# Maofei/loam_velodyne-1

Measured on AMD Instinct MI355X. Metric: scans/sec (odometry+mapping L-M solve) VLP-16 sweep, 1/2/4/8 MI355X, higher is better.
Workload: dtype fp32 (fp64 JtJ accumulation); 1 GPU; config4: independent VLP-16 problems (SR prev+cur, odometry L-M, mapping L-M); problems_per_gpu=1024, global_batch=1024, split=strong, parallelism=shard1

## Files before the change

loam_velodyne-1_amd/csrc/dev_common.hpp:

```cpp
#ifndef LOAM_DEV_COMMON_HPP
#define LOAM_DEV_COMMON_HPP

#include <hip/hip_runtime.h>
#include <stdint.h>

#define LOAM_HD __host__ __device__ __forceinline__
#define LOAM_D __device__ __forceinline__

#ifdef LOAM_BOUNDS_CHECK
#define LOAM_CHECK(cond, a, b)                                                                      \
  do {                                                                                              \
    if (!(cond)) printf("LOAM_CHECK %s:%d %s (%lld, %lld)\n", __FILE__, __LINE__, #cond, (long long)(a), \
                        (long long)(b));                                                            \
  } while (0)
#else
#define LOAM_CHECK(cond, a, b) ((void)0)
#endif

struct PhaseAcc {
  unsigned long long s0, s1, s2;
  unsigned long long sum[2][12];
};
#ifdef LOAM_PHASES
#define LOAM_PH(...) __VA_ARGS__
// ... 251 lines not shown
    mx[d] = b;
  }
  __syncthreads();
}
template <bool HALF = false>
LOAM_D int wave_incl_scan_x(int v) {
  const uint32_t u = (uint32_t)v;
  uint32_t s = u + dpp_u32<kDppShr1>(0u, u);
  s += dpp_u32<kDppShr2>(0u, u);
  s += dpp_u32<kDppShr3>(0u, u);
  s += dpp_u32<kDppShr4, 0xf, 0xe>(0u, s);
  s += dpp_u32<kDppShr8, 0xf, 0xc>(0u, s);
  s += dpp_u32<kDppBcast15, 0xa, 0xf>(0u, s);
  if constexpr (!HALF) s += dpp_u32<kDppBcast31, 0xc, 0xf>(0u, s);
  return (int)s;
}

LOAM_D int wave_incl_max(int v) {
  for (int o = 1; o < 64; o <<= 1) {
    int w = __shfl_up(v, o, 64);
    if (lane_id() >= o) v = max(v, w);
  }
  return v;
}

template <int NT>
LOAM_D int block_incl_max(int v, int* scratch, int& total) {
  const int nw = NT / 64, w = threadIdx.x >> 6, l = lane_id();
  int incl = wave_incl_max(v);
  if (l == 63) scratch[w] = incl;
// ... 1006 lines not shown
```

loam_velodyne-1_amd/csrc/dev_hooks.h:

```cpp
#ifndef LOAM_DEV_HOOKS_H
#define LOAM_DEV_HOOKS_H

#include <stdint.h>

#ifdef __cplusplus
extern "C" {
#endif

typedef struct loam_dev_vg loam_dev_vg;

#define LOAM_DEV_VG_STACK 0
#define LOAM_DEV_VG_CUBES 1
#define LOAM_DEV_VG_SURROUND 2

typedef struct {
  const float* pts;
  int32_t total;
  int32_t nseg;
  const int32_t* begin;
  const int32_t* end;
  const float* leaf;
  const int32_t* nold;
  int32_t route;
  int32_t P;
// ... 43 lines not shown
typedef struct {
  const float* cloud;
  int32_t n_cloud;
  const float* queries;
  int32_t n_queries;
  const int32_t* seeds;
} loam_dev_od_nn_job;

int loam_dev_od_nn_create(int device, loam_dev_od_nn** out);

int loam_dev_od_nn_run(loam_dev_od_nn* h, const loam_dev_od_nn_job* job, uint64_t* lane_key, uint64_t* wave_key,
                       uint64_t* chunk_key, int32_t* left);

int loam_dev_od_nn_destroy(loam_dev_od_nn* h);

#ifdef __cplusplus
}
#endif
#endif
```

loam_velodyne-1_amd/csrc/engine.cpp:

```cpp
#include <hip/hip_runtime.h>

#include <cstdio>
#include <cstddef>
#include <algorithm>
#include <cmath>
#include <cstring>
#include <string>
#include <thread>
#include <vector>

#include "../../include/loam/loam.h"
#include "engine.hpp"
#include "lanes.hpp"
#include "mp.hpp"
#include "od.hpp"
#include "pose_math.hpp"
#include "score.hpp"

#ifdef LOAM_PIPE_TRACE
namespace {
struct PipeTrace {
  struct Mark { int step; const char* stage; hipEvent_t a, b; };
  std::vector<Mark> marks;
  int step = 0;
// ... 71 lines not shown
  return v;
}

}

constexpr size_t kMetaBytes = 8192;

struct loam_ctx {
  loam_config cfg;
  int device = 0;
  hipStream_t st = nullptr;
  int R = 16, cap = 40000;
  int sr_init_count = 0;
  bool sr_inited = false;
  SrBuffers sr1;
  SrBuffers odin;
  OdBuffers od1;
  bool od_inited = false;
  int od_last = 0, od_frame_count = 1;
  float od_sum[6] = {0, 0, 0, 0, 0, 0};
  MpBuffers mp1;
  int map_frame_count = 4;
  bool surround_due = false;
  loamimu::SrQueue* sr_imu = nullptr;
  loamimu::SrQueue* sr_imu_dev = nullptr;
  loamimu::MpQueue mp_imu;
  double imu_last_stamp = -1e300;
  int P = 0;
  SrBuffers srb;
  SrBuffers srb2;
// ... 170 lines not shown
  return LOAM_OK;
}

int sr_errors(int e) {
  if (e & ERR_EMPTY) return fail(LOAM_E_INVAL, "sweep has no finite point");
  if (e & ERR_CAP_RING) return fail(LOAM_E_CAPACITY, "a ring span exceeds the per-ring capacity");
  return LOAM_OK;
}

SrParams sr_params(const loam_ctx* c) {
  SrParams p;
  p.R = c->R;
  p.ring_model = (int)c->cfg.ring_model;
  p.ring_lo = c->cfg.ring_lo_deg;
  p.ring_hi = c->cfg.ring_hi_deg;
  return p;
}

void count_bytes(loam_stats& s) {
  s.bytes_sr = 16 * s.n_raw + 32 * s.n_ring + 16 * (s.n_sharp + s.n_less_sharp + s.n_flat + s.n_less_flat);
  s.bytes_od = 16 * s.od_assoc_points + 16 * s.od_queries + 12 * s.od_queries + 32 * s.od_rows_sum;
  s.bytes_mp = 16 * s.mp_map_points + 96 * s.mp_stack_iters + 64 * s.mp_rows_sum + 32 * s.mp_stack +
               32 * s.mp_map_valid_points;
}

}

namespace loam {
void set_last_error(const std::string& msg) { g_err = msg; }
}
// ... 60 lines not shown
  if (he == hipSuccess) he = hipEventCreateWithFlags(&x->seed_done, hipEventDisableTiming);
  for (auto& e : x->step_done)
    if (he == hipSuccess) he = hipEventCreateWithFlags(&e, hipEventDisableTiming);
  for (auto& e : x->feed_copied)
    if (he == hipSuccess) he = hipEventCreateWithFlags(&e, hipEventDisableTiming);
  x->pin.streams[0] = x->st;
  x->pin.streams[1] = x->st2;
  if (he == hipSuccess) he = hipEventCreateWithFlags(&x->fork, hipEventDisableTiming);
  if (he == hipSuccess) he = hipEventCreateWithFlags(&x->join, hipEventDisableTiming);
  if (he == hipSuccess) he = hipEventCreateWithFlags(&x->fork2, hipEventDisableTiming);
  if (he == hipSuccess) he = hipEventCreateWithFlags(&x->join2, hipEventDisableTiming);
  if (he != hipSuccess) {
    loam_destroy(x);
    return fail(LOAM_E_HIP, std::string("event creation failed: ") + hipGetErrorString(he));
  }
  if (he == hipSuccess) he = sr_alloc(x->sr1, 1, x->cap, x->R);
  if (he == hipSuccess) he = sr_alloc(x->odin, 1, x->cap, x->R);
  if (he == hipSuccess) he = od_alloc(x->od1, 1, x->R, x->cap, (int)c.od_max_iter);
  if (he == hipSuccess) he = mp_alloc(x->mp1, 1, x->R, x->cap, (int)c.map_capacity, (int)c.mp_max_iter);
  x->od1.tune = x->mp1.tune = x->tune;
  if (he == hipSuccess) he = hipMalloc(&x->sr_imu_dev, sizeof(loamimu::SrQueue));
  if (he != hipSuccess) x->sr_imu_dev = nullptr;
  if (he == hipSuccess) he = hipHostMalloc((void**)&x->meta, kMetaBytes, hipHostMallocDefault);
  if (he != hipSuccess) x->meta = nullptr;
  if (he == hipSuccess) he = hipHostMalloc((void**)&x->xb.h, kXferBytes, hipHostMallocCoherent | hipHostMallocMapped);
  if (he != hipSuccess) x->xb.h = nullptr;
  else std::memset(x->xb.h, 0, kXferBytes);
  if (he == hipSuccess) he = hipHostGetDevicePointer((void**)&x->xb.d, x->xb.h, 0);
  x->sr_imu = new loamimu::SrQueue();
  std::memset(x->sr_imu, 0, sizeof(loamimu::SrQueue));
// ... 4 lines not shown
  if (he != hipSuccess) {
    loam_destroy(x);
    return fail(LOAM_E_NOMEM, std::string("device allocation failed: ") + hipGetErrorString(he));
  }
  *out = x;
  return LOAM_OK;
}

void loam_destroy(loam_ctx* x) {
  if (!x) return;
  (void)hipSetDevice(x->device);
  if (x->st) (void)hipStreamSynchronize(x->st);
  if (x->st2) (void)hipStreamSynchronize(x->st2);
  if (x->st3) (void)hipStreamSynchronize(x->st3);
  if (x->st4) (void)hipStreamSynchronize(x->st4);
  sr_free(x->sr1);
  sr_free(x->odin);
  od_free(x->od1);
  mp_free(x->mp1);
  sr_free(x->srb);
  sr_free(x->srb2);
  sr_free(x->srb3);
  od_free(x->odb);
  mp_free(x->mpb);
  mp_free(x->mpb2);
  x->free_feed();
  x->free_pack();
  mp_map_free(x->mio);
  mp_loc_free(x->loc);
  mp_score_free(x->score);
// ... 2113 lines not shown
```

loam_velodyne-1_amd/csrc/engine.hpp:

```cpp
#ifndef LOAM_ENGINE_HPP
#define LOAM_ENGINE_HPP

#include <hip/hip_runtime.h>
#include <stdint.h>

#include <cstring>
#include <string>

#include "../../include/loam/loam.h"
#include "imu.hpp"
#include "prof.hpp"

namespace loam {

enum : int {
  ERR_CAP_RING = 1,
  ERR_CAP_ROWS = 2,
  ERR_EMPTY = 4,
  ERR_CAP_MAP = 8,
  ERR_CAP_STACK = 16,
  ERR_VG_BITS = 32,
};

constexpr int kSrThreads = 512;
// ... 92 lines not shown
  int* err = nullptr;
  int* sel_big = nullptr;
  int* sel_list = nullptr;
  int* st_loff = nullptr;
  uint64_t* big_keys = nullptr;
  int* big_sidx = nullptr;
  int* big_cand = nullptr;
  int big_stride = 0;
  __host__ __device__ int ntiles() const { return (cap + kSrThreads - 1) / kSrThreads; }
};

struct SrParams {
  int R;
  int ring_model;
  float ring_lo, ring_hi;
  loamimu::SrQueue* imu = nullptr;
  double time_scan = 0.0;
  const loamimu::LaneHdr* imu_lane = nullptr;
  loamimu::SrTail* imu_tail = nullptr;
  int* imu_tile_key = nullptr;
};

struct DevAlloc {
  hipError_t err = hipSuccess;
  template <class T>
  void operator()(T** p, size_t bytes) {
    *p = nullptr;
    if (err != hipSuccess) return;
    void* q = nullptr;
    err = hipMalloc(&q, bytes ? bytes : 16);
// ... 61 lines not shown
  }
  void finish() {
    for (int i = 0; i < nout; ++i) memcpy(out[i].dst, out[i].src, out[i].bytes);
    nout = 0;
  }
  void release() {
    if (buf) (void)hipHostFree(buf);
    buf = nullptr;
    cap = off = 0;
    nout = 0;
  }
};

void set_last_error(const std::string& msg);

hipError_t sr_alloc(SrBuffers& b, int S, int cap, int R);
hipError_t sr_scatter_packed(const float4* src, const int* off, const int* n, float4* raw, int cap, int S,
                             hipStream_t st);
void sr_free(SrBuffers& b);
constexpr int kPackClouds = 5;
hipError_t sr_pack_offsets(const SrBuffers& b, int s0, int ns, uint64_t* table, hipStream_t st);
hipError_t sr_pack(const SrBuffers& b, const uint64_t* table, int s0, int ns, int j0, int nj, unsigned clouds,
                   const long long* dbase, float4* dst, hipStream_t st);
void sr_launch(const SrBuffers& b, const SrParams& p, hipStream_t st, Prof* prof = nullptr,
               hipEvent_t sorted = nullptr);

}

#endif
```

loam_velodyne-1_amd/csrc/sr.hip:

```cpp
#include <type_traits>

#include "dev_common.hpp"
#include "engine.hpp"

using namespace loamdev;

namespace loam {

namespace {


LOAM_D int ring_id(const SrParams& p, float angle) {
  if (p.ring_model == LOAM_RING_LINEAR) {
    const float step = (p.ring_hi - p.ring_lo) / (float)(p.R - 1);
    const float angleID = (angle - p.ring_lo) / step;
    return (int)(angleID + 0.5f);
  }
  int rounded = (int)(D(angle) + (D(angle) < 0.0 ? -0.5 : +0.5));
  return rounded > 0 ? rounded : rounded + (p.R - 1);
}

LOAM_D int ring_of(const SrParams& p, float px, float py, float pz) {
  const float af = atanf(py / sqrtf(px * px + pz * pz)) * 57.2957795f;
  const int lo = ring_id(p, af - 1e-3f), hi = ring_id(p, af + 1e-3f);
  if (lo == hi) return lo;
  return ring_id(p, (float)(atan(D(py) / sqrt(D(px * px + pz * pz))) * 180 / M_PI));
}

using loamimu::kNoOri;
using loamimu::ori_first;
using loamimu::ori_key;
using loamimu::ori_second;
LOAM_D bool finite3(const float4& q) {
  return isfinite(q.x) && isfinite(q.y) && isfinite(q.z);
}

template <bool IMU>
__global__ __launch_bounds__(kSrThreads) void k_sr_ring_sort(SrBuffers b, SrParams p) {
  const int s = blockIdx.x, tid = threadIdx.x, lane = lane_id(), w = tid >> 6;
  const int n = b.raw_n[s];
  const float4* raw = b.raw + (size_t)s * b.cap;
  float* tori = b.tmp_ori + (size_t)s * b.cap;
  uint8_t* tsid = b.tmp_sid + (size_t)s * b.cap;
  const int R = p.R, ntiles = (n + kSrThreads - 1) / kSrThreads;
  int* tc = b.tilecnt + (size_t)s * b.ntiles() * R;
  __shared__ int sh_first, sh_last, sh_F, sh_total;
  __shared__ float sh_start, sh_end;
  __shared__ int sh_cnt[64];
  __shared__ int sh_wcnt[kSrThreads / 64][64];
  __shared__ int sh_base[64];
  if (tid == 0) { sh_first = 0x7fffffff; sh_last = -1; sh_F = 0x7fffffff; }
  __syncthreads();
  int f = 0x7fffffff, l = -1;
  for (int i = tid; i < n; i += kSrThreads) {
    if (finite3(raw[i])) { f = min(f, i); l = max(l, i); }
  }
  f = wave_min_i(f);
  l = wave_max_i(l);
  if (lane == 0) { atomicMin(&sh_first, f); atomicMax(&sh_last, l); }
  __syncthreads();
  if (sh_last < 0) {
    if (tid == 0) { b.n_full[s] = 0; b.err[s] |= ERR_EMPTY; }
    return;
  }
  if (tid == 0) {
// ... 6 lines not shown
    sh_end = endOri;
  }
  __syncthreads();
  const float startOri = sh_start, endOri = sh_end;
  int Floc = 0x7fffffff;
  for (int t = 0; t < ntiles; ++t) {
    if (tid < R) sh_cnt[tid] = 0;
    __syncthreads();
    const int i = t * kSrThreads + tid;
    if (i < n) {
      const float4 q = raw[i];
      uint8_t sid = 255;
      float ori = 0.0f;
      if (finite3(q)) {
        const float px = q.y, py = q.z, pz = q.x;
        int scanID = ring_of(p, px, py, pz);
        if (scanID >= 0 && scanID <= R - 1) {
          sid = (uint8_t)scanID;
          ori = -atan2f_fdlibm(px, pz);
          float o1 = ori_first(ori, startOri);
          if (D(o1 - startOri) > M_PI) Floc = min(Floc, i);
          atomicAdd(&sh_cnt[scanID], 1);
        }
      }
      tori[i] = ori;
      tsid[i] = sid;
    }
    __syncthreads();
    if (tid < R) tc[t * R + tid] = sh_cnt[tid];
    __syncthreads();
  }
// ... 58 lines not shown
        const float ori = (i <= F) ? ori_first(tori[i], startOri) : ori_second(tori[i], endOri);
        const float relTime = (ori - startOri) / (endOri - startOri);
        pointTime = (float)(D(relTime) * 0.1);
        g = loamimu::first_later(*imu, front0, p.time_scan + pointTime);
      }
      int tmax;
      const int incl = block_incl_max<kSrThreads>(g, sh_imuscr, tmax);
      front_i = max(sh_carry, incl);
      __syncthreads();
      if (tid == 0) sh_carry = max(sh_carry, tmax);
    }
    loamimu::Cur cur;
    float fs[6];
    if (lane < R) sh_wcnt[w][lane] = 0;
    __builtin_amdgcn_wave_barrier();
    int rank = 0;
    uint64_t mval = __ballot(valid);
    while (mval) {
      const int leader = __ffsll((unsigned long long)mval) - 1;
      const int rl = __builtin_amdgcn_readlane(sid, leader);
      const uint64_t mm = __ballot(valid && sid == rl);
      if (valid && sid == rl) rank = __popcll(mm & lanemask_lt());
      if (lane == leader) sh_wcnt[w][rl] = __popcll(mm);
      mval &= ~mm;
    }
    __syncthreads();
    if (valid) {
      int pos = sh_base[sid] + tc[t * R + sid] + rank;
      for (int v = 0; v < w; ++v) pos += sh_wcnt[v][sid];
      const float4 q = raw[i];
      float ori = tori[i];
      ori = (i <= F) ? ori_first(ori, startOri) : ori_second(ori, endOri);
      float relTime = (ori - startOri) / (endOri - startOri);
      float4 o;
      o.x = q.y;
      o.y = q.z;
      o.z = q.x;
      o.w = (float)(sid + 0.1 * D(relTime));
      if (imu) {
        cur = loamimu::interpolate(*imu, (front0 + front_i) % loamimu::kQue, p.time_scan, pointTime);
// ... 67 lines not shown
    for (int base = 0; base < n; base += 64) {
      const int i = base + lane;
      const uint64_t m = __ballot(i < n && finite3(raw[i]));
      if (m) { f = base + __ffsll((unsigned long long)m) - 1; break; }
    }
    if (lane == 0) sh_first = f;
  } else if (w == 1) {
    int l = -1;
    for (int base = n - 1; base >= 0; base -= 64) {
      const int i = base - lane;
      const uint64_t m = __ballot(i >= 0 && finite3(raw[i]));
      if (m) { l = base - (__ffsll((unsigned long long)m) - 1); break; }
    }
    if (lane == 0) sh_last = l;
  }
  if (tid < R) sh_cnt[tid] = 0;
  if (tid == 0) sh_F = 0x7fffffff;
  __syncthreads();
  if (tid == 0) sh_start = sh_last >= 0 ? -atan2f_fdlibm(raw[sh_first].y, raw[sh_first].x) : 0.0f;
  if (tid == 64 && (t == 0 || imu) && sh_last >= 0) sh_end_raw = -atan2f_fdlibm(raw[sh_last].y, raw[sh_last].x);
  __syncthreads();
  const float startOri = sh_start;
  if (IMU && imu) {
    if (tid == 0) {
      float endOri = 0.0f;
      if (sh_last >= 0) {
        endOri = (float)(D(sh_end_raw) + 2 * M_PI);
        if (D(endOri - startOri) > 3 * M_PI) endOri = (float)(D(endOri) - 2 * M_PI);
        else if (D(endOri - startOri) < M_PI) endOri = (float)(D(endOri) + 2 * M_PI);
      }
// ... 14 lines not shown
    }
    b.sweep_ori[2 * s] = startOri;
    b.sweep_ori[2 * s + 1] = endOri;
  }
  int Floc = 0x7fffffff;
  int k1[kRingE], k2[kRingE];
#pragma unroll
  for (int e = 0; e < kRingE; ++e) {
    const int i = t * kRingTile + e * kSrThreads + tid;
    k1[e] = k2[e] = kNoOri;
    if (i < n) {
      uint8_t sid = 255;
      float ori = 0.0f;
      if (finite3(q[e])) {
        const float px = q[e].y, py = q[e].z, pz = q[e].x;
        const int scanID = ring_of(p, px, py, pz);
        if (scanID >= 0 && scanID <= R - 1) {
          sid = (uint8_t)scanID;
          ori = -atan2f_fdlibm(px, pz);
          const float o1 = ori_first(ori, startOri);
          if (D(o1 - startOri) > M_PI) Floc = min(Floc, i);
          atomicAdd(&sh_cnt[scanID], 1);
          if (IMU && imu) {
            k1[e] = ori_key(o1);
            k2[e] = ori_key(ori_second(ori, sh_end));
          }
        }
      }
      b.tmp_ori[(size_t)s * b.cap + i] = ori;
      b.tmp_sid[(size_t)s * b.cap + i] = sid;
    }
// ... 13 lines not shown
      else m2 = max(m2, k2[e]);
    }
    m1 = wave_max_i(m1); m2 = wave_max_i(m2); m3 = wave_max_i(m3);
    if (lane == 0) { atomicMax(&sh_key[0], m1); atomicMax(&sh_key[1], m2); atomicMax(&sh_key[2], m3); }
    __syncthreads();
    if (tid < 3) p.imu_tile_key[((size_t)s * b.ntiles() + t) * 3 + tid] = sh_key[tid];
  }
}

template <bool IMU>
__global__ __launch_bounds__(kSrThreads) void k_sr_ring_scatter(SrBuffers b, SrParams p) {
  constexpr int kW = kSrThreads / 64, kSlots = kRingE * kW;
  static_assert(kSlots <= 64 && (kSlots & (kSlots - 1)) == 0, "slot scan width");
  const int s = blockIdx.y, t = blockIdx.x, tid = threadIdx.x, lane = lane_id(), w = tid >> 6;
  const int n = b.raw_n[s], R = p.R, nt = (n + kRingTile - 1) / kRingTile;
  if (t >= (nt > 0 ? nt : 1)) return;
  const bool imu = IMU && p.imu_lane[s].has != 0;
  __shared__ int sh_later;
  __shared__ int sh_tot[64], sh_pre[64], sh_base[64], sh_F;
  __shared__ int sh_wcnt[64][kSlots];
  int sid[kRingE], rank[kRingE];
  float4 q[kRingE];
  float ori[kRingE];
#pragma unroll
  for (int e = 0; e < kRingE; ++e) {
    const int i = t * kRingTile + e * kSrThreads + tid;
    sid[e] = 255;
    q[e] = make_float4(0, 0, 0, 0);
    ori[e] = 0.0f;
    if (i < n) {
// ... 11 lines not shown
  for (int k = tid; k < nt * R; k += kSrThreads) {
    const int v = tc[k];
    if (v) {
      atomicAdd(&sh_tot[k % R], v);
      if (k / R < t) atomicAdd(&sh_pre[k % R], v);
      if (IMU && k / R > t) sh_later = 1;
    }
  }
  int F = 0x7fffffff;
  for (int k = tid; k < nt; k += kSrThreads) F = min(F, b.tileF[(size_t)s * b.ntiles() + k]);
  F = wave_min_i(F);
  if (lane == 0 && F != 0x7fffffff) atomicMin(&sh_F, F);
#pragma unroll
  for (int e = 0; e < kRingE; ++e) {
    const bool valid = sid[e] != 255;
    rank[e] = 0;
    uint64_t mval = __ballot(valid);
    while (mval) {
      const int leader = __ffsll((unsigned long long)mval) - 1;
      const int rl = __builtin_amdgcn_readlane(sid[e], leader);
      const uint64_t mm = __ballot(valid && sid[e] == rl);
      if (valid && sid[e] == rl) rank[e] = __popcll(mm & lanemask_lt());
      if (lane == leader) sh_wcnt[rl][e * kW + w] = __popcll(mm);
      mval &= ~mm;
    }
  }
  __syncthreads();
  if (tid == 0) {
    int run = 0;
    for (int r = 0; r < R; ++r) { sh_base[r] = run; run += sh_tot[r]; }
    if (t == 0) {
      b.n_full[s] = run;
      if (n <= 0) b.err[s] |= ERR_EMPTY;
    }
  }
  for (int k = tid; k < R * kSlots; k += kSrThreads) {
    const int r = k / kSlots, j = k % kSlots;
    const int v = sh_wcnt[r][j];
    int incl = v;
#pragma unroll
// ... 103 lines not shown
}

#ifndef LOAM_SR_RING_FUSED
#define LOAM_SR_RING_FUSED 1
#endif
constexpr bool kSrRingFused = LOAM_SR_RING_FUSED;
constexpr int kSrRingFusedMin = 64;
__global__ __launch_bounds__(kSrThreads) void k_sr_ring_fused(SrBuffers b, SrParams p, int rtiles) {
  constexpr int kW = kSrThreads / 64, kSlots = kRingE * kW;
  static_assert(kSlots <= 64 && (kSlots & (kSlots - 1)) == 0, "slot scan width");
  const int tid = threadIdx.x, lane = lane_id(), w = tid >> 6;
  __shared__ int sh_ticket, sh_last, sh_F;
  __shared__ float sh_start, sh_end_raw;
  __shared__ int sh_cnt[64], sh_tot[64], sh_pre[64], sh_base[64];
  __shared__ int sh_wcnt[64][kSlots];
  if (tid == 0) sh_ticket = atomicAdd(&b.ring_sync[0], 1);
  __syncthreads();
  const int s = sh_ticket / rtiles, t = sh_ticket % rtiles;
  const int n = b.raw_n[s], R = p.R, nt = (n + kRingTile - 1) / kRingTile;
  if (t == 0) {
    if (tid < 2 * R) b.ring_se[s * 2 * R + tid] = 0;
    if (tid == 0) b.err[s] = 0;
  }
  if (n <= 0) {
    if (t == 0 && tid == 0) {
      b.n_full[s] = 0;
      b.err[s] |= ERR_EMPTY;
    }
    return;
  }
  if (t >= nt) return;
  const float4* raw = b.raw + (size_t)s * b.cap;
  float4 q[kRingE];
#pragma unroll
// ... 14 lines not shown
        f = w == 0 ? k + src : n - 1 - k - src;
        v.x = __shfl(v.x, src, 64);
        v.y = __shfl(v.y, src, 64);
        break;
      }
    }
    if (lane == 0) {
      if (w == 0) {
        sh_start = f >= 0 ? -atan2f_fdlibm(v.y, v.x) : 0.0f;
      } else {
        sh_last = f;
        if (f >= 0) sh_end_raw = -atan2f_fdlibm(v.y, v.x);
      }
    }
  }
  if (tid < R) sh_cnt[tid] = 0;
  if (tid == 0) sh_F = 0x7fffffff;
  for (int k = tid; k < 64 * kSlots; k += kSrThreads) (&sh_wcnt[0][0])[k] = 0;
  __syncthreads();
  const float startOri = sh_start;
  float endOri = 0.0f;
  if (sh_last >= 0) {
    endOri = (float)(D(sh_end_raw) + 2 * M_PI);
    if (D(endOri - startOri) > 3 * M_PI) endOri = (float)(D(endOri) - 2 * M_PI);
    else if (D(endOri - startOri) < M_PI) endOri = (float)(D(endOri) + 2 * M_PI);
  }
  if (tid == 0 && t == 0) {
    if (sh_last < 0) b.err[s] |= ERR_EMPTY;
    b.sweep_ori[2 * s] = startOri;
    b.sweep_ori[2 * s + 1] = endOri;
  }
  int sid[kRingE], rank[kRingE];
  float ori[kRingE];
  int Floc = 0x7fffffff;
#pragma unroll
  for (int e = 0; e < kRingE; ++e) {
    const int i = t * kRingTile + e * kSrThreads + tid;
    sid[e] = 255;
    ori[e] = 0.0f;
    if (i < n && finite3(q[e])) {
      const float px = q[e].y, py = q[e].z, pz = q[e].x;
      const int scanID = ring_of(p, px, py, pz);
      if (scanID >= 0 && scanID <= R - 1) {
        sid[e] = scanID;
        ori[e] = -atan2f_fdlibm(px, pz);
        if (D(ori_first(ori[e], startOri) - startOri) > M_PI) Floc = min(Floc, i);
        atomicAdd(&sh_cnt[scanID], 1);
      }
    }
  }
  Floc = wave_min_i(Floc);
  if (lane == 0 && Floc != 0x7fffffff) atomicMin(&sh_F, Floc);
  __syncthreads();
  if (tid < R) __hip_atomic_store(&b.tilecnt[((size_t)s * rtiles + t) * R + tid], sh_cnt[tid], __ATOMIC_RELAXED, __HIP_MEMORY_SCOPE_AGENT);
  if (tid == 0) __hip_atomic_store(&b.tileF[(size_t)s * rtiles + t], sh_F, __ATOMIC_RELAXED, __HIP_MEMORY_SCOPE_AGENT);
#pragma unroll
  for (int e = 0; e < kRingE; ++e) {
    const bool valid = sid[e] != 255;
    rank[e] = 0;
    uint64_t mval = __ballot(valid);
    while (mval) {
      const int leader = __ffsll((unsigned long long)mval) - 1;
      const int rl = __builtin_amdgcn_readlane(sid[e], leader);
      const uint64_t mm = __ballot(valid && sid[e] == rl);
      if (valid && sid[e] == rl) rank[e] = __popcll(mm & lanemask_lt());
      if (lane == leader) sh_wcnt[rl][e * kW + w] = __popcll(mm);
      mval &= ~mm;
    }
  }
  if (tid < R) { sh_tot[tid] = 0; sh_pre[tid] = 0; }
  __syncthreads();
  for (int k = tid; k < R * kSlots; k += kSrThreads) {
    const int r = k / kSlots, j = k % kSlots;
    const int v = sh_wcnt[r][j];
    int incl = v;
#pragma unroll
    for (int o = 1; o < kSlots; o <<= 1) {
      const int u = __shfl_up(incl, o, kSlots);
      if (j >= o) incl += u;
    }
    sh_wcnt[r][j] = incl - v;
  }
  const int* tc = b.tilecnt + (size_t)s * rtiles * R;
  for (int k = tid; k < nt * R; k += kSrThreads) {
    int v;
    while ((v = __hip_atomic_load(&tc[k], __ATOMIC_RELAXED, __HIP_MEMORY_SCOPE_AGENT)) < 0) __builtin_amdgcn_s_sleep(1);
// ... 2 lines not shown
      if (k / R < t) atomicAdd(&sh_pre[k % R], v);
    }
  }
  int F = 0x7fffffff;
  for (int k = tid; k < nt; k += kSrThreads) {
    int v;
    while ((v = __hip_atomic_load(&b.tileF[(size_t)s * rtiles + k], __ATOMIC_RELAXED, __HIP_MEMORY_SCOPE_AGENT)) < 0)
      __builtin_amdgcn_s_sleep(1);
    F = min(F, v);
  }
  F = wave_min_i(F);
  if (tid == 0) sh_F = 0x7fffffff;
  __syncthreads();
  if (lane == 0 && F != 0x7fffffff) atomicMin(&sh_F, F);
  __syncthreads();
  if (tid == 0) {
    int run = 0;
    for (int r = 0; r < R; ++r) { sh_base[r] = run; run += sh_tot[r]; }
    if (t == 0) b.n_full[s] = run;
  }
  __syncthreads();
  F = sh_F;
#pragma unroll
  for (int e = 0; e < kRingE; ++e) {
    const int i = t * kRingTile + e * kSrThreads + tid;
    if (sid[e] != 255) {
      const int pos = sh_base[sid[e]] + sh_pre[sid[e]] + sh_wcnt[sid[e]][e * kW + w] + rank[e];
      const float o = (i <= F) ? ori_first(ori[e], startOri) : ori_second(ori[e], endOri);
      const float relTime = (o - startOri) / (endOri - startOri);
      b.full[(size_t)s * b.cap + pos] = make_float4(q[e].y, q[e].z, q[e].x, (float)(sid[e] + 0.1 * D(relTime)));
    }
  }
}

constexpr int kFeatTile = 256;
constexpr int kFeatE = 4;
constexpr int kFeatSpan = kFeatTile * kFeatE;

__global__ __launch_bounds__(kFeatTile) void k_sr_features(SrBuffers b, SrParams p) {
  const int s = blockIdx.y, tid = threadIdx.x;
  if ((blockIdx.x | blockIdx.y) == 0 && tid < 2) b.sel_list[tid] = 0;
  const int n = b.n_full[s];
  const int i0 = blockIdx.x * kFeatSpan;
  if (i0 >= n) return;
  const float4* pts = b.full + (size_t)s * b.cap;
  __shared__ float4 sp[kFeatSpan + 12];
  __shared__ int8_t evt[kFeatSpan + 12];
  for (int t = tid; t < kFeatSpan + 12; t += kFeatTile) {
    int g = i0 - 6 + t;
    if (g >= 0 && g < n) sp[t] = pts[g];
  }
  __syncthreads();
  for (int t = tid; t < kFeatSpan + 11; t += kFeatTile) {
    const int k = i0 - 6 + t;
    int8_t e = 0;
    if (k >= 5 && k <= n - 7) {
      const float4 a = sp[t], c = sp[t + 1];
      float dX = c.x - a.x, dY = c.y - a.y, dZ = c.z - a.z;
      float diff = dX * dX + dY * dY + dZ * dZ;
      if (D(diff) > 0.1) {
        float depth1 = (float)sqrt(D(a.x * a.x + a.y * a.y + a.z * a.z));
        float depth2 = (float)sqrt(D(c.x * c.x + c.y * c.y + c.z * c.z));
        if (depth1 > depth2) {
          dX = c.x - a.x * depth2 / depth1;
          dY = c.y - a.y * depth2 / depth1;
          dZ = c.z - a.z * depth2 / depth1;
          if (sqrt(D(dX * dX + dY * dY + dZ * dZ)) / D(depth2) < 0.1) e = 1;
        } else {
          dX = c.x * depth1 / depth2 - a.x;
          dY = c.y * depth1 / depth2 - a.y;
          dZ = c.z * depth1 / depth2 - a.z;
          if (sqrt(D(dX * dX + dY * dY + dZ * dZ)) / D(depth1) < 0.1) e = 2;
        }
      }
    }
    evt[t] = e;
  }
  __syncthreads();
#pragma unroll
  for (int fe = 0; fe < kFeatE; ++fe) {
    const int i = i0 + fe * kFeatTile + tid;
    if (i >= n) return;
    const int li = fe * kFeatTile + tid + 6;
    const size_t gi = (size_t)s * b.cap + i;
    float cv = 0.0f;
    if (i >= 5 && i < n - 5) {
      const float4* q = sp + li;
      float dX = q[-5].x + q[-4].x + q[-3].x + q[-2].x + q[-1].x - 10 * q[0].x + q[1].x + q[2].x +
                 q[3].x + q[4].x + q[5].x;
      float dY = q[-5].y + q[-4].y + q[-3].y + q[-2].y + q[-1].y - 10 * q[0].y + q[1].y + q[2].y +
                 q[3].y + q[4].y + q[5].y;
      float dZ = q[-5].z + q[-4].z + q[-3].z + q[-2].z + q[-1].z - 10 * q[0].z + q[1].z + q[2].z +
                 q[3].z + q[4].z + q[5].z;
      cv = dX * dX + dY * dY + dZ * dZ;
      const int v = (int)q[0].w;
      const int pv = (i == 5) ? -1 : (int)q[-1].w;
      if (v != pv && v > 0 && v < p.R) {
        atomicMax(&b.ring_se[s * 2 * p.R + v], i + 5);
        atomicMax(&b.ring_se[s * 2 * p.R + p.R + v - 1], i - 5);
      }
    }
    int pk = 0;
    for (int k = 0; k <= 5; ++k) pk |= (evt[li + k] == 1);
    for (int k = 1; k <= 6; ++k) pk |= (evt[li - k] == 2);
    if (i >= 5 && i <= n - 7) {
      const float4 a = sp[li - 1], c = sp[li], e = sp[li + 1];
      float dX = e.x - c.x, dY = e.y - c.y, dZ = e.z - c.z;
      float diff = dX * dX + dY * dY + dZ * dZ;
      float dX2 = c.x - a.x, dY2 = c.y - a.y, dZ2 = c.z - a.z;
      float diff2 = dX2 * dX2 + dY2 * dY2 + dZ2 * dZ2;
      float dis = c.x * c.x + c.y * c.y + c.z * c.z;
      if (D(diff) > 0.0002 * D(dis) && D(diff2) > 0.0002 * D(dis)) pk = 1;
    }
    int gap = 0;
    if (i >= 1) {
      const float4 a = sp[li], c = sp[li - 1];
      const float ex = a.x - c.x, ey = a.y - c.y, ez = a.z - c.z;
      gap = D(ex * ex + ey * ey + ez * ez) > 0.05 ? 1 : 0;
    }
    b.curv[gi] = cv;
    b.picked[gi] = (uint8_t)(pk | (gap << 1));
  }
}

template <int CAP, bool SIDX>
struct SelShared {
  uint64_t keys[CAP];
  int sidx[SIDX ? CAP : 1];
  uint16_t cand[CAP];
  uint8_t pk[CAP + 16];
  int8_t lab[CAP + 16];
// ... 1022 lines not shown
  A(&b.flat, (size_t)S * R * kFlatPerRing * sizeof(float4));
  A(&b.lflat, n * sizeof(float4));
  A(&b.cnt, (size_t)S * 4 * sizeof(int));
  A(&b.err, S * sizeof(int));
  A(&b.sel_big, S * sizeof(int));
  A(&b.sel_list, (2 + 2 * (size_t)S) * sizeof(int));
  A(&b.st_loff, (size_t)S * R * sizeof(int));
  b.big_stride = next_pow2(cap);
  A(&b.big_keys, (size_t)kBigSlots * b.big_stride * sizeof(uint64_t));
  A(&b.big_sidx, (size_t)kBigSlots * b.big_stride * sizeof(int));
  A(&b.big_cand, (size_t)kBigSlots * b.big_stride * sizeof(int));
  if (A.err != hipSuccess) sr_free(b);
  return A.err;
}

void sr_free(SrBuffers& b) {
  void* ptrs[] = {b.raw, b.raw_n, b.tmp_ori, b.tmp_sid, b.tilecnt, b.tileF, b.ring_sync, b.sweep_ori, b.full, b.n_full, b.curv,
                  b.picked, b.sortind, b.label, b.ring_se, b.st_sharp, b.st_lsharp, b.st_flat,
                  b.st_lflat, b.st_cnt, b.st_cand, b.st_ncand, b.sharp, b.lsharp, b.flat, b.lflat, b.cnt, b.err, b.sel_big, b.sel_list, b.st_loff, b.big_keys, b.big_sidx, b.big_cand};
  for (void* q : ptrs)
    if (q) HIPCHK(hipFree(q));
  b = SrBuffers();
}

int sr_ring_fused_capacity() {
  static int cap[64];
  int dev = 0;
  if (hipGetDevice(&dev) != hipSuccess || dev < 0 || dev >= 64) return 0;
  if (cap[dev] == 0) {
    int per_cu = 0, cus = 0;
// ... 33 lines not shown
  }
  mark("k_sr_ring_sort");
  if (sorted) HIPCHK(hipEventRecord(sorted, st));
  hipLaunchKernelGGL(k_sr_features, dim3((b.cap + kFeatSpan - 1) / kFeatSpan, b.S), dim3(kFeatTile), 0,
                     st, b, p);
  mark("k_sr_features");
  hipLaunchKernelGGL(k_sr_pick, dim3((b.R + kPickWaves - 1) / kPickWaves, b.S), dim3(64 * kPickWaves), 0, st, b, p);
  hipLaunchKernelGGL(k_sr_ringvg, dim3(b.R, b.S), dim3(kSelThreads), LOAM_RINGVG_PAD, st, b, p);
  hipLaunchKernelGGL((k_sr_select<kRingCap, 1>), dim3(b.R, std::min(b.S, kSelListGrid)), dim3(kSelThreads), 0, st, b, p);
  hipLaunchKernelGGL((k_sr_select<16, 2>), dim3(kBigSlots), dim3(kSelThreads), 0, st, b, p);
  mark("k_sr_select");
  hipLaunchKernelGGL(k_sr_compact, dim3(b.R, b.S), dim3(256), 0, st, b, p);
  mark("k_sr_compact");
}

}
```

Baseline: 95770 scans/s.

## Use precomputed ring-boundary table and bitwise ballot ranking in scan registration

Adds a host-built table of tangent-space ring boundaries so each point's ring ID comes from a cheap polynomial atan estimate and a table lookup, falling back to the exact atan path only near boundaries. Replaces the per-distinct-ring leader loop for in-wave ranking with a fixed number of bitwise ballots over the ring-key bits. It also caches LDS point loads into registers in the feature kernel and adds optional phase timing and a device test hook. The intent is to cut transcendental and serialized ballot cost in the ring sort. The price is extra shared-memory table loads and some host-side table construction complexity.

After: 97150 scans/s (median of 6 runs). +1.4%, better.

```diff
diff --git a/loam_velodyne-1_amd/csrc/dev_common.hpp b/loam_velodyne-1_amd/csrc/dev_common.hpp
--- a/loam_velodyne-1_amd/csrc/dev_common.hpp
+++ b/loam_velodyne-1_amd/csrc/dev_common.hpp
@@ -289,6 +289,25 @@
   s += dpp_u32<kDppBcast15, 0xa, 0xf>(0u, s);
   if constexpr (!HALF) s += dpp_u32<kDppBcast31, 0xc, 0xf>(0u, s);
   return (int)s;
+}
+
+LOAM_D int wave_key_rank(int key, bool valid, int nb, int& peers) {
+  uint64_t m = __ballot(valid);
+#pragma unroll
+  for (int b = 0; b < 6; ++b) {
+    if (b < nb) {
+      const bool bit = (key >> b) & 1;
+      const uint64_t bal = __ballot(bit);
+      m &= bit ? bal : ~bal;
+    }
+  }
+  peers = __popcll(m);
+  return __popcll(m & lanemask_lt());
+}
+LOAM_HD int key_bits(int R) {
+  int nb = 0;
+  while ((1 << nb) < R) ++nb;
+  return nb;
 }
 
 LOAM_D int wave_incl_max(int v) {
diff --git a/loam_velodyne-1_amd/csrc/dev_hooks.h b/loam_velodyne-1_amd/csrc/dev_hooks.h
--- a/loam_velodyne-1_amd/csrc/dev_hooks.h
+++ b/loam_velodyne-1_amd/csrc/dev_hooks.h
@@ -81,6 +81,10 @@
 
 int loam_dev_od_nn_destroy(loam_dev_od_nn* h);
 
+#define LOAM_DEV_SR_RING_MAX (1 << 22)
+int loam_dev_sr_ring_of(int device, int32_t n_rings, int32_t ring_model, float ring_lo_deg, float ring_hi_deg,
+                        const float* pts, int32_t n, int32_t* ring, int32_t* exact, int32_t* fast);
+
 #ifdef __cplusplus
 }
 #endif
diff --git a/loam_velodyne-1_amd/csrc/engine.cpp b/loam_velodyne-1_amd/csrc/engine.cpp
--- a/loam_velodyne-1_amd/csrc/engine.cpp
+++ b/loam_velodyne-1_amd/csrc/engine.cpp
@@ -109,6 +109,7 @@
   int sr_init_count = 0;
   bool sr_inited = false;
   SrBuffers sr1;
+  SrRingTab ring_tab;
   SrBuffers odin;
   OdBuffers od1;
   bool od_inited = false;
@@ -309,6 +310,7 @@
   p.ring_model = (int)c->cfg.ring_model;
   p.ring_lo = c->cfg.ring_lo_deg;
   p.ring_hi = c->cfg.ring_hi_deg;
+  c->ring_tab.fill(p);
   return p;
 }
 
@@ -399,6 +401,7 @@
     loam_destroy(x);
     return fail(LOAM_E_HIP, std::string("event creation failed: ") + hipGetErrorString(he));
   }
+  if (he == hipSuccess) he = sr_ring_tab_alloc(x->ring_tab, sr_params(x));
   if (he == hipSuccess) he = sr_alloc(x->sr1, 1, x->cap, x->R);
   if (he == hipSuccess) he = sr_alloc(x->odin, 1, x->cap, x->R);
   if (he == hipSuccess) he = od_alloc(x->od1, 1, x->R, x->cap, (int)c.od_max_iter);
@@ -433,6 +436,7 @@
   if (x->st2) (void)hipStreamSynchronize(x->st2);
   if (x->st3) (void)hipStreamSynchronize(x->st3);
   if (x->st4) (void)hipStreamSynchronize(x->st4);
+  sr_ring_tab_free(x->ring_tab);
   sr_free(x->sr1);
   sr_free(x->odin);
   od_free(x->od1);
diff --git a/loam_velodyne-1_amd/csrc/engine.hpp b/loam_velodyne-1_amd/csrc/engine.hpp
--- a/loam_velodyne-1_amd/csrc/engine.hpp
+++ b/loam_velodyne-1_amd/csrc/engine.hpp
@@ -130,6 +130,9 @@
   int R;
   int ring_model;
   float ring_lo, ring_hi;
+  const float4* ring_tab = nullptr;
+  int ring_n = 0;
+  float ring_a0 = 0.0f, ring_ainv = 0.0f;
   loamimu::SrQueue* imu = nullptr;
   double time_scan = 0.0;
   const loamimu::LaneHdr* imu_lane = nullptr;
@@ -221,6 +224,19 @@
 
 void set_last_error(const std::string& msg);
 
+struct SrRingTab {
+  float4* dev = nullptr;
+  int n = 0;
+  float a0 = 0.0f, ainv = 0.0f;
+  void fill(SrParams& p) const {
+    p.ring_tab = dev;
+    p.ring_n = dev ? n : 0;
+    p.ring_a0 = a0;
+    p.ring_ainv = ainv;
+  }
+};
+hipError_t sr_ring_tab_alloc(SrRingTab& t, const SrParams& p);
+void sr_ring_tab_free(SrRingTab& t);
 hipError_t sr_alloc(SrBuffers& b, int S, int cap, int R);
 hipError_t sr_scatter_packed(const float4* src, const int* off, const int* n, float4* raw, int cap, int S,
                              hipStream_t st);
diff --git a/loam_velodyne-1_amd/csrc/sr.hip b/loam_velodyne-1_amd/csrc/sr.hip
--- a/loam_velodyne-1_amd/csrc/sr.hip
+++ b/loam_velodyne-1_amd/csrc/sr.hip
@@ -1,16 +1,33 @@
+#include <cmath>
 #include <type_traits>
+#include <vector>
 
 #include "dev_common.hpp"
+#include "dev_hooks.h"
 #include "engine.hpp"
 
 using namespace loamdev;
 
 namespace loam {
 
+#ifdef LOAM_SR_PHASES
+__device__ unsigned long long g_sr_ph[8];
+#define SR_PH(k)                                                                  \
+  do {                                                                            \
+    if (threadIdx.x == 0) {                                                       \
+      const unsigned long long now = __builtin_amdgcn_s_memrealtime();            \
+      ph_t[k] = now - ph_last;                                                    \
+      ph_last = now;                                                              \
+    }                                                                             \
+  } while (0)
+#else
+#define SR_PH(k) ((void)0)
+#endif
+
 namespace {
 
 
-LOAM_D int ring_id(const SrParams& p, float angle) {
+LOAM_HD int ring_id(const SrParams& p, float angle) {
   if (p.ring_model == LOAM_RING_LINEAR) {
     const float step = (p.ring_hi - p.ring_lo) / (float)(p.R - 1);
     const float angleID = (angle - p.ring_lo) / step;
@@ -20,11 +37,35 @@
   return rounded > 0 ? rounded : rounded + (p.R - 1);
 }
 
-LOAM_D int ring_of(const SrParams& p, float px, float py, float pz) {
+LOAM_D int ring_of_exact(const SrParams& p, float px, float py, float pz) {
   const float af = atanf(py / sqrtf(px * px + pz * pz)) * 57.2957795f;
   const int lo = ring_id(p, af - 1e-3f), hi = ring_id(p, af + 1e-3f);
   if (lo == hi) return lo;
   return ring_id(p, (float)(atan(D(py) / sqrt(D(px * px + pz * pz))) * 180 / M_PI));
+}
+
+#ifndef LOAM_SR_RING_TAB
+#define LOAM_SR_RING_TAB 1
+#endif
+LOAM_D int ring_of(const SrParams& p, const float4* tab, float px, float py, float pz, bool* fast = nullptr) {
+  const float r2 = px * px + pz * pz;
+  if (fast) *fast = false;
+  if (LOAM_SR_RING_TAB && p.ring_n > 0 && r2 >= 1e-30f && r2 <= 3e38f) {
+    const float t = py * __builtin_amdgcn_rsqf(r2);
+    const float t2 = t * t;
+    const float a = t * fmaf(t2, fmaf(t2, fmaf(t2, -1.0f / 7, 0.2f), -1.0f / 3), 1.0f) * 57.2957795f;
+    const float g = fminf(fmaxf((a - p.ring_a0) * p.ring_ainv, 0.0f), (float)(p.ring_n - 1));
+    const float4 e = tab[(int)g];
+    if (t > e.x && t < e.y) {
+      if (fast) *fast = true;
+      return __float_as_int(e.z);
+    }
+  }
+  return ring_of_exact(p, px, py, pz);
+}
+constexpr int kRingTabMax = 64;
+LOAM_D void ring_tab_load(const SrParams& p, float4* tab) {
+  if ((int)threadIdx.x < p.ring_n) tab[threadIdx.x] = p.ring_tab[threadIdx.x];
 }
 
 using loamimu::kNoOri;
@@ -43,12 +84,15 @@
   float* tori = b.tmp_ori + (size_t)s * b.cap;
   uint8_t* tsid = b.tmp_sid + (size_t)s * b.cap;
   const int R = p.R, ntiles = (n + kSrThreads - 1) / kSrThreads;
+  const int nb = key_bits(R);
   int* tc = b.tilecnt + (size_t)s * b.ntiles() * R;
   __shared__ int sh_first, sh_last, sh_F, sh_total;
   __shared__ float sh_start, sh_end;
   __shared__ int sh_cnt[64];
   __shared__ int sh_wcnt[kSrThreads / 64][64];
   __shared__ int sh_base[64];
+  __shared__ float4 sh_rtab[kRingTabMax];
+  ring_tab_load(p, sh_rtab);
   if (tid == 0) { sh_first = 0x7fffffff; sh_last = -1; sh_F = 0x7fffffff; }
   __syncthreads();
   int f = 0x7fffffff, l = -1;
@@ -85,7 +129,7 @@
       float ori = 0.0f;
       if (finite3(q)) {
         const float px = q.y, py = q.z, pz = q.x;
-        int scanID = ring_of(p, px, py, pz);
+        int scanID = ring_of(p, sh_rtab, px, py, pz);
         if (scanID >= 0 && scanID <= R - 1) {
           sid = (uint8_t)scanID;
           ori = -atan2f_fdlibm(px, pz);
@@ -174,16 +218,9 @@
     float fs[6];
     if (lane < R) sh_wcnt[w][lane] = 0;
     __builtin_amdgcn_wave_barrier();
-    int rank = 0;
-    uint64_t mval = __ballot(valid);
-    while (mval) {
-      const int leader = __ffsll((unsigned long long)mval) - 1;
-      const int rl = __builtin_amdgcn_readlane(sid, leader);
-      const uint64_t mm = __ballot(valid && sid == rl);
-      if (valid && sid == rl) rank = __popcll(mm & lanemask_lt());
-      if (lane == leader) sh_wcnt[w][rl] = __popcll(mm);
-      mval &= ~mm;
-    }
+    int peers;
+    const int rank = wave_key_rank(sid, valid, nb, peers);
+    if (valid && rank == 0) sh_wcnt[w][sid] = peers;
     __syncthreads();
     if (valid) {
       int pos = sh_base[sid] + tc[t * R + sid] + rank;
@@ -281,6 +318,8 @@
     }
     if (lane == 0) sh_last = l;
   }
+  __shared__ float4 sh_rtab[kRingTabMax];
+  ring_tab_load(p, sh_rtab);
   if (tid < R) sh_cnt[tid] = 0;
   if (tid == 0) sh_F = 0x7fffffff;
   __syncthreads();
@@ -325,7 +364,7 @@
       float ori = 0.0f;
       if (finite3(q[e])) {
         const float px = q[e].y, py = q[e].z, pz = q[e].x;
-        const int scanID = ring_of(p, px, py, pz);
+        const int scanID = ring_of(p, sh_rtab, px, py, pz);
         if (scanID >= 0 && scanID <= R - 1) {
           sid = (uint8_t)scanID;
           ori = -atan2f_fdlibm(px, pz);
@@ -369,6 +408,7 @@
   static_assert(kSlots <= 64 && (kSlots & (kSlots - 1)) == 0, "slot scan width");
   const int s = blockIdx.y, t = blockIdx.x, tid = threadIdx.x, lane = lane_id(), w = tid >> 6;
   const int n = b.raw_n[s], R = p.R, nt = (n + kRingTile - 1) / kRingTile;
+  const int nb = key_bits(R);
   if (t >= (nt > 0 ? nt : 1)) return;
   const bool imu = IMU && p.imu_lane[s].has != 0;
   __shared__ int sh_later;
@@ -410,16 +450,9 @@
 #pragma unroll
   for (int e = 0; e < kRingE; ++e) {
     const bool valid = sid[e] != 255;
-    rank[e] = 0;
-    uint64_t mval = __ballot(valid);
-    while (mval) {
-      const int leader = __ffsll((unsigned long long)mval) - 1;
-      const int rl = __builtin_amdgcn_readlane(sid[e], leader);
-      const uint64_t mm = __ballot(valid && sid[e] == rl);
-      if (valid && sid[e] == rl) rank[e] = __popcll(mm & lanemask_lt());
-      if (lane == leader) sh_wcnt[rl][e * kW + w] = __popcll(mm);
-      mval &= ~mm;
-    }
+    int peers;
+    rank[e] = wave_key_rank(sid[e], valid, nb, peers);
+    if (valid && rank[e] == 0) sh_wcnt[sid[e]][e * kW + w] = peers;
   }
   __syncthreads();
   if (tid == 0) {
@@ -553,10 +586,15 @@
   __shared__ float sh_start, sh_end_raw;
   __shared__ int sh_cnt[64], sh_tot[64], sh_pre[64], sh_base[64];
   __shared__ int sh_wcnt[64][kSlots];
+#ifdef LOAM_SR_PHASES
+  unsigned long long ph_t[8] = {0}, ph_last = __builtin_amdgcn_s_memrealtime();
+#endif
   if (tid == 0) sh_ticket = atomicAdd(&b.ring_sync[0], 1);
   __syncthreads();
+  SR_PH(1);
   const int s = sh_ticket / rtiles, t = sh_ticket % rtiles;
   const int n = b.raw_n[s], R = p.R, nt = (n + kRingTile - 1) / kRingTile;
+  const int nb = key_bits(R);
   if (t == 0) {
     if (tid < 2 * R) b.ring_se[s * 2 * R + tid] = 0;
     if (tid == 0) b.err[s] = 0;
@@ -601,10 +639,13 @@
       }
     }
   }
+  __shared__ float4 sh_rtab[kRingTabMax];
+  ring_tab_load(p, sh_rtab);
   if (tid < R) sh_cnt[tid] = 0;
   if (tid == 0) sh_F = 0x7fffffff;
   for (int k = tid; k < 64 * kSlots; k += kSrThreads) (&sh_wcnt[0][0])[k] = 0;
   __syncthreads();
+  SR_PH(2);
   const float startOri = sh_start;
   float endOri = 0.0f;
   if (sh_last >= 0) {
@@ -627,7 +668,7 @@
     ori[e] = 0.0f;
     if (i < n && finite3(q[e])) {
       const float px = q[e].y, py = q[e].z, pz = q[e].x;
-      const int scanID = ring_of(p, px, py, pz);
+      const int scanID = ring_of(p, sh_rtab, px, py, pz);
       if (scanID >= 0 && scanID <= R - 1) {
         sid[e] = scanID;
         ori[e] = -atan2f_fdlibm(px, pz);
@@ -639,24 +680,19 @@
   Floc = wave_min_i(Floc);
   if (lane == 0 && Floc != 0x7fffffff) atomicMin(&sh_F, Floc);
   __syncthreads();
+  SR_PH(3);
   if (tid < R) __hip_atomic_store(&b.tilecnt[((size_t)s * rtiles + t) * R + tid], sh_cnt[tid], __ATOMIC_RELAXED, __HIP_MEMORY_SCOPE_AGENT);
   if (tid == 0) __hip_atomic_store(&b.tileF[(size_t)s * rtiles + t], sh_F, __ATOMIC_RELAXED, __HIP_MEMORY_SCOPE_AGENT);
 #pragma unroll
   for (int e = 0; e < kRingE; ++e) {
     const bool valid = sid[e] != 255;
-    rank[e] = 0;
-    uint64_t mval = __ballot(valid);
-    while (mval) {
-      const int leader = __ffsll((unsigned long long)mval) - 1;
-      const int rl = __builtin_amdgcn_readlane(sid[e], leader);
-      const uint64_t mm = __ballot(valid && sid[e] == rl);
-      if (valid && sid[e] == rl) rank[e] = __popcll(mm & lanemask_lt());
-      if (lane == leader) sh_wcnt[rl][e * kW + w] = __popcll(mm);
-      mval &= ~mm;
-    }
+    int peers;
+    rank[e] = wave_key_rank(sid[e], valid, nb, peers);
+    if (valid && rank[e] == 0) sh_wcnt[sid[e]][e * kW + w] = peers;
   }
   if (tid < R) { sh_tot[tid] = 0; sh_pre[tid] = 0; }
   __syncthreads();
+  SR_PH(4);
   for (int k = tid; k < R * kSlots; k += kSrThreads) {
     const int r = k / kSlots, j = k % kSlots;
     const int v = sh_wcnt[r][j];
@@ -689,12 +725,14 @@
   __syncthreads();
   if (lane == 0 && F != 0x7fffffff) atomicMin(&sh_F, F);
   __syncthreads();
+  SR_PH(5);
   if (tid == 0) {
     int run = 0;
     for (int r = 0; r < R; ++r) { sh_base[r] = run; run += sh_tot[r]; }
     if (t == 0) b.n_full[s] = run;
   }
   __syncthreads();
+  SR_PH(6);
   F = sh_F;
 #pragma unroll
   for (int e = 0; e < kRingE; ++e) {
@@ -706,12 +744,24 @@
       b.full[(size_t)s * b.cap + pos] = make_float4(q[e].y, q[e].z, q[e].x, (float)(sid[e] + 0.1 * D(relTime)));
     }
   }
+#ifdef LOAM_SR_PHASES
+  SR_PH(7);
+  if (tid == 0) {
+    atomicAdd(&g_sr_ph[0], 1ull);
+    for (int k = 1; k < 8; ++k) atomicAdd(&g_sr_ph[k], ph_t[k]);
+  }
+#endif
 }
 
 constexpr int kFeatTile = 256;
 constexpr int kFeatE = 4;
 constexpr int kFeatSpan = kFeatTile * kFeatE;
 
+LOAM_D float4 lds_point(const float4* p) {
+  float4 v = *p;
+  asm volatile("" : "+v"(v.w));
+  return v;
+}
 __global__ __launch_bounds__(kFeatTile) void k_sr_features(SrBuffers b, SrParams p) {
   const int s = blockIdx.y, tid = threadIdx.x;
   if ((blockIdx.x | blockIdx.y) == 0 && tid < 2) b.sel_list[tid] = 0;
@@ -730,7 +780,7 @@
     const int k = i0 - 6 + t;
     int8_t e = 0;
     if (k >= 5 && k <= n - 7) {
-      const float4 a = sp[t], c = sp[t + 1];
+      const float4 a = lds_point(sp + t), c = lds_point(sp + t + 1);
       float dX = c.x - a.x, dY = c.y - a.y, dZ = c.z - a.z;
       float diff = dX * dX + dY * dY + dZ * dZ;
       if (D(diff) > 0.1) {
@@ -760,7 +810,10 @@
     const size_t gi = (size_t)s * b.cap + i;
     float cv = 0.0f;
     if (i >= 5 && i < n - 5) {
-      const float4* q = sp + li;
+      float4 qv[11];
+#pragma unroll
+      for (int k = 0; k < 11; ++k) qv[k] = lds_point(sp + li - 5 + k);
+      const float4* q = qv + 5;
       float dX = q[-5].x + q[-4].x + q[-3].x + q[-2].x + q[-1].x - 10 * q[0].x + q[1].x + q[2].x +
                  q[3].x + q[4].x + q[5].x;
       float dY = q[-5].y + q[-4].y + q[-3].y + q[-2].y + q[-1].y - 10 * q[0].y + q[1].y + q[2].y +
@@ -779,7 +832,7 @@
     for (int k = 0; k <= 5; ++k) pk |= (evt[li + k] == 1);
     for (int k = 1; k <= 6; ++k) pk |= (evt[li - k] == 2);
     if (i >= 5 && i <= n - 7) {
-      const float4 a = sp[li - 1], c = sp[li], e = sp[li + 1];
+      const float4 a = lds_point(sp + li - 1), c = lds_point(sp + li), e = lds_point(sp + li + 1);
       float dX = e.x - c.x, dY = e.y - c.y, dZ = e.z - c.z;
       float diff = dX * dX + dY * dY + dZ * dZ;
       float dX2 = c.x - a.x, dY2 = c.y - a.y, dZ2 = c.z - a.z;
@@ -789,7 +842,7 @@
     }
     int gap = 0;
     if (i >= 1) {
-      const float4 a = sp[li], c = sp[li - 1];
+      const float4 a = lds_point(sp + li), c = lds_point(sp + li - 1);
       const float ex = a.x - c.x, ey = a.y - c.y, ez = a.z - c.z;
       gap = D(ex * ex + ey * ey + ez * ez) > 0.05 ? 1 : 0;
     }
@@ -1842,6 +1895,95 @@
   return A.err;
 }
 
+static std::vector<float4> sr_ring_tab_build(const SrParams& p, float& a0, float& ainv) {
+  std::vector<float4> none;
+  if (p.R < 1) return none;
+  if (p.ring_model == LOAM_RING_LINEAR) {
+    const float step = (p.ring_hi - p.ring_lo) / (float)(p.R - 1);
+    if (!(step >= 0.01f) || !(fabsf(p.ring_lo) <= 1e4f) || !(fabsf(p.ring_hi) <= 1e4f)) return none;
+  }
+  constexpr int G = 128;
+  std::vector<float> last_old, first_new;
+  std::vector<int> val;
+  float a = -89.0f;
+  int va = ring_id(p, a);
+  val.push_back(va);
+  for (int i = 1; i <= 178 * G; ++i) {
+    const float c = -89.0f + (float)i / G;
+    const int vc = ring_id(p, c);
+    if (vc != va) {
+      float lo = a, hi = c;
+      for (;;) {
+        const float mid = lo + (hi - lo) * 0.5f;
+        if (!(mid > lo && mid < hi)) break;
+        if (ring_id(p, mid) == va) lo = mid; else hi = mid;
+      }
+      if (ring_id(p, hi) != vc) return none;
+      last_old.push_back(lo);
+      first_new.push_back(hi);
+      val.push_back(vc);
+    }
+    a = c;
+    va = vc;
+  }
+  const int nbnd = (int)first_new.size();
+  int i0 = -1, i1 = -1;
+  for (int i = 1; i <= nbnd - 1; ++i)
+    if (val[i] >= 0 && val[i] <= p.R - 1) {
+      if (i0 < 0) i0 = i;
+      i1 = i;
+    }
+  if (i0 < 0 || i1 - i0 + 1 > kRingTabMax) return none;
+  const int n = i1 - i0 + 1;
+  auto tan_deg = [](double deg) { return tan(deg * M_PI / 180.0); };
+  std::vector<float4> tab(n);
+  for (int k = 0; k < n; ++k) {
+    const int i = i0 + k;
+    const double dlo = tan_deg(D(first_new[i - 1]) + 1e-3), dhi = tan_deg(D(last_old[i]) - 1e-3);
+    float flo = (float)dlo, fhi = (float)dhi;
+    if (D(flo) < dlo) flo = nextafterf(flo, INFINITY);
+    if (D(fhi) > dhi) fhi = nextafterf(fhi, -INFINITY);
+    flo = nextafterf(flo, INFINITY);
+    fhi = nextafterf(fhi, -INFINITY);
+    tab[k] = make_float4(flo, fhi, __builtin_bit_cast(float, val[i]), 0.0f);
+  }
+  for (int skip = 0; skip < 2 && skip < n; ++skip) {
+    const float top = first_new[i1], w = (top - first_new[i0 - 1 + skip]) / (float)(n - skip);
+    a0 = top - (float)n * w;
+    ainv = 1.0f / w;
+    bool ok = w > 0.0f;
+    for (int k = 0; k < n && ok; ++k) {
+      const float mid = 0.5f * (first_new[i0 + k - 1] + first_new[i0 + k]);
+      ok = (int)fminf(fmaxf((mid - a0) * ainv, 0.0f), (float)(n - 1)) == k;
+    }
+    if (ok) return tab;
+  }
+  return none;
+}
+
+hipError_t sr_ring_tab_alloc(SrRingTab& t, const SrParams& p) {
+  t = SrRingTab();
+  const std::vector<float4> tab = sr_ring_tab_build(p, t.a0, t.ainv);
+  if (tab.empty()) return hipSuccess;
+  hipError_t e = hipMalloc((void**)&t.dev, tab.size() * sizeof(float4));
+  if (e != hipSuccess) {
+    t.dev = nullptr;
+    return e;
+  }
+  e = hipMemcpy(t.dev, tab.data(), tab.size() * sizeof(float4), hipMemcpyHostToDevice);
+  if (e != hipSuccess) {
+    sr_ring_tab_free(t);
+    return e;
+  }
+  t.n = (int)tab.size();
+  return hipSuccess;
+}
+
+void sr_ring_tab_free(SrRingTab& t) {
+  if (t.dev) HIPCHK(hipFree(t.dev));
+  t = SrRingTab();
+}
+
 void sr_free(SrBuffers& b) {
   void* ptrs[] = {b.raw, b.raw_n, b.tmp_ori, b.tmp_sid, b.tilecnt, b.tileF, b.ring_sync, b.sweep_ori, b.full, b.n_full, b.curv,
                   b.picked, b.sortind, b.label, b.ring_se, b.st_sharp, b.st_lsharp, b.st_flat,
@@ -1905,4 +2047,68 @@
   mark("k_sr_compact");
 }
 
-}
+namespace {
+__global__ __launch_bounds__(256) void k_dev_sr_ring_of(SrParams p, const float4* pts, int n, int* ring, int* exact,
+                                                         int* fast) {
+  __shared__ float4 sh_rtab[kRingTabMax];
+  ring_tab_load(p, sh_rtab);
+  __syncthreads();
+  const int i = blockIdx.x * 256 + threadIdx.x;
+  if (i >= n) return;
+  const float4 q = pts[i];
+  const float px = q.y, py = q.z, pz = q.x;
+  bool f;
+  ring[i] = ring_of(p, sh_rtab, px, py, pz, &f);
+  exact[i] = ring_of_exact(p, px, py, pz);
+  fast[i] = f ? 1 : 0;
+}
+}
+
+}
+
+extern "C" int loam_dev_sr_ring_of(int device, int32_t n_rings, int32_t ring_model, float ring_lo_deg,
+                                   float ring_hi_deg, const float* pts, int32_t n, int32_t* ring, int32_t* exact,
+                                   int32_t* fast) {
+  using namespace loam;
+  if (!pts || !ring || !exact || !fast || n < 1 || n > LOAM_DEV_SR_RING_MAX) return LOAM_E_INVAL;
+  if (n_rings < 2 || n_rings > 64 || (ring_model != LOAM_RING_VLP16 && ring_model != LOAM_RING_LINEAR)) return LOAM_E_INVAL;
+  int ndev = 0;
+  if (hipGetDeviceCount(&ndev) != hipSuccess || ndev == 0) return LOAM_E_HIP;
+  if (device < 0 || device >= ndev) return LOAM_E_INVAL;
+  if (hipSetDevice(device) != hipSuccess) return LOAM_E_HIP;
+  SrParams p;
+  p.R = n_rings;
+  p.ring_model = ring_model;
+  p.ring_lo = ring_lo_deg;
+  p.ring_hi = ring_hi_deg;
+  SrRingTab tab;
+  float4* dpts = nullptr;
+  int* dout = nullptr;
+  hipError_t e = sr_ring_tab_alloc(tab, p);
+  if (e == hipSuccess) e = hipMalloc((void**)&dpts, (size_t)n * sizeof(float4));
+  if (e == hipSuccess) e = hipMalloc((void**)&dout, 3 * (size_t)n * sizeof(int));
+  const bool nomem = e == hipErrorOutOfMemory;
+  if (e == hipSuccess) e = hipMemcpy(dpts, pts, (size_t)n * sizeof(float4), hipMemcpyHostToDevice);
+  if (e == hipSuccess) {
+    tab.fill(p);
+    hipLaunchKernelGGL(k_dev_sr_ring_of, dim3((n + 255) / 256), dim3(256), 0, nullptr, p, dpts, n, dout, dout + n,
+                       dout + 2 * (size_t)n);
+    e = hipGetLastError();
+  }
+  if (e == hipSuccess) e = hipMemcpy(ring, dout, (size_t)n * sizeof(int), hipMemcpyDeviceToHost);
+  if (e == hipSuccess) e = hipMemcpy(exact, dout + n, (size_t)n * sizeof(int), hipMemcpyDeviceToHost);
+  if (e == hipSuccess) e = hipMemcpy(fast, dout + 2 * (size_t)n, (size_t)n * sizeof(int), hipMemcpyDeviceToHost);
+  if (dpts) (void)hipFree(dpts);
+  if (dout) (void)hipFree(dout);
+  sr_ring_tab_free(tab);
+  return e == hipSuccess ? LOAM_OK : (nomem ? LOAM_E_NOMEM : LOAM_E_HIP);
+}
+
+#ifdef LOAM_SR_PHASES
+extern "C" int loam_debug_phases_sr(unsigned long long* out) {
+  if (hipDeviceSynchronize() != hipSuccess) return -1;
+  if (hipMemcpyFromSymbol(out, HIP_SYMBOL(loam::g_sr_ph), sizeof(loam::g_sr_ph)) != hipSuccess) return -1;
+  const unsigned long long zero[8] = {0};
+  return hipMemcpyToSymbol(HIP_SYMBOL(loam::g_sr_ph), zero, sizeof(zero)) == hipSuccess ? 0 : -1;
+}
+#endif
```
